# mll-lab-nu/TStar

Measured on AMD Instinct MI355X. Metric: candidate frames scored/sec (whole node) + sec/video to 8 keyframes, 1h@1fps, higher is better.
Workload: dtype f32 held exactly as 3 bf16 terms per operand: every GEMM and vision-attention operand (activations, weights, Q, K, V, softmax probabilities) = three round-to-nearest bf16 terms carrying all 24 significand bits; the 6 partial products with i + j <= 2 (each exact) on v_mfma_f32_32x32x16_bf16, f32 accu

## Files before the change

tstar_amd/csrc/gemm_f32.hip:

```cpp
#include "common.h"
#include "kernels.h"
#include "prof.h"
#include <type_traits>
#include <utility>

namespace tstar {

constexpr int BK = 32, LDS_LD = BK + 4;

__device__ __forceinline__ void tile_mn(int tile, int mt, int nt, int gm, int& mi, int& ni) {
    if (gm <= 1) { mi = tile / nt; ni = tile - mi * nt; return; }
    const int per = gm * nt;
    const int sp = tile / per, r = tile - sp * per;
    const int left = mt - sp * gm;
    const int rows = left < gm ? left : gm;
    ni = r / rows;
    mi = sp * gm + (r - ni * rows);
}

__device__ __forceinline__ float epi_act(float v, int act) {
    if (act == ACT_QGELU) return v * __builtin_amdgcn_rcpf(1.0f + __builtin_amdgcn_exp2f(-1.702f * 1.44269504088896340736f * v));
    if (act == ACT_GELU) return 0.5f * v * (1.0f + erff(v * 0.70710678118654752440f));
    return v;
}

template <int TM_, int TN_, int MINW_>
struct Cfg { static constexpr int TM = TM_, TN = TN_, MINW = MINW_, BM = 2 * TM_ * 32, BN = 2 * TN_ * 32; };
using Cfg128 = Cfg<2, 2, 2>;
using Cfg64N = Cfg<1, 2, 2>;
using Cfg64 = Cfg<1, 1, 4>;
using Cfg128W = Cfg<2, 4, 2>;

template <class CF, int ACT, bool HAS_BIAS, bool HAS_RES, bool PATCH, bool GUARD>
__device__ __forceinline__ void gemm_epilogue_impl(const GemmArgs& g, f32x16 (&acc)[CF::TM][CF::TN], const int m0, const int n0,
                                                   const int wm, const int wn, const int l31, const int h) {
    constexpr int TM = CF::TM, TN = CF::TN;
#pragma unroll
    for (int j = 0; j < TN; ++j) {
        const int col = n0 + wn * TN * 32 + j * 32 + l31;
        const float bv = HAS_BIAS ? g.bias[col] : 0.f;
#pragma unroll
        for (int i = 0; i < TM; ++i) {
            const int rbase = m0 + wm * TM * 32 + i * 32 + 4 * h;
            size_t off[16];
            float extra[16];
#pragma unroll
            for (int r = 0; r < 16; ++r) {
                int row = rbase + (r & 3) + 8 * (r >> 2);
                if (GUARD) row = row < g.M ? row : g.M - 1;
                size_t orow = row;
                float e = 0.f;
                if (PATCH) {
                    const int b = row / g.patch_np, p = row - b * g.patch_np;
                    orow = (size_t)b * (g.patch_np + 1) + 1 + p;
                    e = g.pos[(size_t)(1 + p) * g.N + col];
                }
                off[r] = orow * g.ldc + col;
                if (HAS_RES) e += g.res[off[r]];
                extra[r] = e;
            }
            float v[16];
#pragma unroll
            for (int r = 0; r < 16; ++r) {
                v[r] = epi_act(acc[i][j][r] + bv, ACT);
                if (PATCH || HAS_RES) v[r] += extra[r];
            }
#pragma unroll
            for (int r = 0; r < 16; ++r) {
                if (!GUARD || rbase + (r & 3) + 8 * (r >> 2) < g.M) g.C[off[r]] = v[r];
            }
        }
    }
}

template <class CF, int ACT, bool HAS_BIAS, bool HAS_RES, bool PATCH, bool GUARD>
__device__ __forceinline__ void gemm_epilogue_wide(const GemmArgs& g, f32x16 (&acc)[CF::TM][CF::TN], const int m0, const int n0,
                                                   const int wm, const int wn, const int l31, const int h) {
    constexpr int TM = CF::TM, TN = CF::TN;
#pragma unroll
    for (int i = 0; i < TM; ++i) {
        const int rbase = m0 + wm * TM * 32 + i * 32 + 4 * h;
        unsigned roff[16], poff[PATCH ? 16 : 1];
#pragma unroll
        for (int r = 0; r < 16; ++r) {
            int row = rbase + (r & 3) + 8 * (r >> 2);
            if (GUARD) row = row < g.M ? row : g.M - 1;
            unsigned orow = (unsigned)row;
            if (PATCH) {
                const int b = row / g.patch_np, p = row - b * g.patch_np;
                orow = (unsigned)(b * (g.patch_np + 1) + 1 + p);
                poff[r] = (unsigned)(1 + p) * (unsigned)g.N;
            }
            roff[r] = orow * (unsigned)g.ldc;
        }
#pragma unroll
        for (int j = 0; j < TN; ++j) {
            const int col = n0 + wn * TN * 32 + j * 32 + l31;
            const float bv = HAS_BIAS ? g.bias[col] : 0.f;
            float e[16];
#pragma unroll
            for (int r = 0; r < 16; ++r) {
                float x = 0.f;
                if (PATCH) x = g.pos[(size_t)poff[r] + col];
                if (HAS_RES) x += g.res[(size_t)roff[r] + col];
                e[r] = x;
            }
#pragma unroll
            for (int r = 0; r < 16; ++r) {
                float v = epi_act(acc[i][j][r] + bv, ACT);
                if (PATCH || HAS_RES) v += e[r];
                e[r] = v;
            }
#pragma unroll
            for (int r = 0; r < 16; ++r) {
                if (!GUARD || rbase + (r & 3) + 8 * (r >> 2) < g.M) g.C[(size_t)roff[r] + col] = e[r];
            }
            __builtin_amdgcn_sched_barrier(0);
        }
    }
}

template <class CF, int ACT, bool HAS_BIAS, bool HAS_RES, bool PATCH>
__device__ __forceinline__ void gemm_epilogue(const GemmArgs& g, f32x16 (&acc)[CF::TM][CF::TN], const int m0, const int n0,
                                              const int wm, const int wn, const int l31, const int h) {
    if constexpr (CF::TN >= 4) {
        if (m0 + CF::BM <= g.M) gemm_epilogue_wide<CF, ACT, HAS_BIAS, HAS_RES, PATCH, false>(g, acc, m0, n0, wm, wn, l31, h);
        else gemm_epilogue_wide<CF, ACT, HAS_BIAS, HAS_RES, PATCH, true>(g, acc, m0, n0, wm, wn, l31, h);
        return;
    }
    if (m0 + CF::BM <= g.M) gemm_epilogue_impl<CF, ACT, HAS_BIAS, HAS_RES, PATCH, false>(g, acc, m0, n0, wm, wn, l31, h);
    else gemm_epilogue_impl<CF, ACT, HAS_BIAS, HAS_RES, PATCH, true>(g, acc, m0, n0, wm, wn, l31, h);
}

typedef __bf16 bf16x8 __attribute__((ext_vector_type(8)));
typedef unsigned int u32x4 __attribute__((ext_vector_type(4)));
typedef unsigned int u32x2 __attribute__((ext_vector_type(2)));

__device__ __forceinline__ int bfw_off(int row, int chunk) { return row * 64 + ((chunk ^ ((row >> 2) & 3)) << 4); }

__device__ __forceinline__ void split4_bf16x3(const f32x4 v, u32x2 (&out)[3]) {
    unsigned t[3][4];
#pragma unroll
    for (int e = 0; e < 4; ++e) {
        float r = v[e];
#pragma unroll
        for (int k = 0; k < 3; ++k) {
            const unsigned b = __float_as_uint(r) & 0xFFFF0000u;
            t[k][e] = b;
            r = r - __uint_as_float(b);
        }
    }
#pragma unroll
    for (int k = 0; k < 3; ++k) {
        out[k][0] = (t[k][0] >> 16) | t[k][1];
        out[k][1] = (t[k][2] >> 16) | t[k][3];
    }
}

typedef __bf16 bf16x2 __attribute__((ext_vector_type(2)));
typedef float f32x2 __attribute__((ext_vector_type(2)));
__device__ __forceinline__ void split4_bf16x2(const f32x4 v, u32x2 (&out)[2]) {
#pragma unroll
    for (int p = 0; p < 2; ++p) {
        f32x2 x; x[0] = v[2 * p]; x[1] = v[2 * p + 1];
        const bf16x2 hi = __builtin_convertvector(x, bf16x2);
        const unsigned hb = __builtin_bit_cast(unsigned, hi);
        f32x2 r;
        r[0] = x[0] - __uint_as_float(hb << 16);
        r[1] = x[1] - __uint_as_float(hb & 0xFFFF0000u);
        const bf16x2 lo = __builtin_convertvector(r, bf16x2);
        out[0][p] = hb;
        out[1][p] = __builtin_bit_cast(unsigned, lo);
    }
}

template <class CF, int WMODE, int ACT, bool HAS_BIAS, bool HAS_RES, bool PATCH>
__device__ __forceinline__ void gemm_tile_bf16w(const GemmArgs& g, const int m0, const int n0, float* smem_f) {
    constexpr int TM = CF::TM, TN = CF::TN, BM = CF::BM, BN = CF::BN;
    constexpr int NAT = WMODE == GEMM_W_BF16_EXACT ? 3 : 2, NWT = 1;
    constexpr int NPROD = WMODE == GEMM_W_BF16_2T ? 2 : 3;
    constexpr int DEPTH = TN >= 4 ? 1 : 2;
    constexpr int A_T = BM * 64, W_T = BN * 64, BUF = NAT * A_T + NWT * W_T;
    char* smem = reinterpret_cast<char*>(smem_f);
    const int t = threadIdx.x;
    const int lane = t & 63, wave = t >> 6;
    const int wm = wave >> 1, wn = wave & 1;
    const int l31 = lane & 31, h = lane >> 5;
    constexpr int NA = BM / 32, NB = BN / 64;
    const int c4 = t & 7, r0 = t >> 3;
    const int wc = t & 3, wr = t >> 2;
    const float* ap[NA];
    size_t bo[NB];
#pragma unroll
    for (int i = 0; i < NA; ++i) {
        int ar = m0 + r0 + 32 * i;
        ar = ar < g.M ? ar : g.M - 1;
        ap[i] = g.A + (size_t)ar * g.lda + c4 * 4;
    }
#pragma unroll
    for (int i = 0; i < NB; ++i) bo[i] = (size_t)(n0 + wr + 64 * i) * g.K + wc * 8;

    f32x16 acc[TM][TN];
#pragma unroll
    for (int i = 0; i < TM; ++i)
#pragma unroll
        for (int j = 0; j < TN; ++j)
#pragma unroll
            for (int r = 0; r < 16; ++r) acc[i][j][r] = 0.f;

    f32x4 ra[DEPTH][NA];
    u32x4 rb[DEPTH][NWT][NB];
    auto gload = [&](auto SET, int kt) __attribute__((always_inline)) {
        constexpr int st = decltype(SET)::value;
#pragma unroll
        for (int i = 0; i < NA; ++i) ra[st][i] = *reinterpret_cast<const f32x4*>(ap[i] + kt * BK);
#pragma unroll
        for (int i = 0; i < NB; ++i) {
            rb[st][0][i] = *reinterpret_cast<const u32x4*>(g.Wb + bo[i] + kt * BK);
        }
    };
    auto lstore = [&](auto SET, int buf) __attribute__((always_inline)) {
        constexpr int st = decltype(SET)::value;
        char* base = smem + buf * BUF;
#pragma unroll
        for (int i = 0; i < NA; ++i) {
            u32x2 sp[NAT];
            if constexpr (WMODE == GEMM_W_BF16_EXACT) split4_bf16x3(ra[st][i], sp);
            else split4_bf16x2(ra[st][i], sp);
            const int off = bfw_off(r0 + 32 * i, c4 >> 1) + (c4 & 1) * 8;
#pragma unroll
            for (int k = 0; k < NAT; ++k) *reinterpret_cast<u32x2*>(base + k * A_T + off) = sp[k];
        }
#pragma unroll
        for (int w = 0; w < NWT; ++w)
#pragma unroll
            for (int i = 0; i < NB; ++i)
                *reinterpret_cast<u32x4*>(base + NAT * A_T + w * W_T + bfw_off(wr + 64 * i, wc)) = rb[st][w][i];
    };
    auto compute = [&](int buf) __attribute__((always_inline)) {
        const char* base = smem + buf * BUF;
        __builtin_amdgcn_s_setprio(1);
#pragma unroll
        for (int s = 0; s < 2; ++s) {
            bf16x8 fa[NAT][TM], fw[NWT][TN];
#pragma unroll
            for (int k = 0; k < NAT; ++k)
#pragma unroll
                for (int i = 0; i < TM; ++i)
                    fa[k][i] = *reinterpret_cast<const bf16x8*>(base + k * A_T + bfw_off(wm * TM * 32 + i * 32 + l31, 2 * s + h));
#pragma unroll
            for (int w = 0; w < NWT; ++w)
#pragma unroll
                for (int j = 0; j < TN; ++j)
                    fw[w][j] = *reinterpret_cast<const bf16x8*>(base + NAT * A_T + w * W_T + bfw_off(wn * TN * 32 + j * 32 + l31, 2 * s + h));
#pragma unroll
            for (int p = NPROD - 1; p >= 0; --p) {
                const int ka = p, kw = 0;
#pragma unroll
                for (int i = 0; i < TM; ++i)
#pragma unroll
                    for (int j = 0; j < TN; ++j)
                        acc[i][j] = __builtin_amdgcn_mfma_f32_32x32x16_bf16(fa[ka][i], fw[kw][j], acc[i][j], 0, 0, 0);
            }
        }
        __builtin_amdgcn_s_setprio(0);
    };
    using S0 = std::integral_constant<int, 0>;
    using S1 = std::integral_constant<int, DEPTH - 1>;
    const int nk = g.K / BK;
    if constexpr (DEPTH == 1) {
        gload(S0{}, 0);
        lstore(S0{}, 0);
        __syncthreads();
        for (int kt = 0; kt < nk; ++kt) {
            const bool more = kt + 1 < nk;
            if (more) gload(S0{}, kt + 1);
            compute(kt & 1);
            if (more) lstore(S0{}, (kt + 1) & 1);
            __syncthreads();
        }
        gemm_epilogue<CF, ACT, HAS_BIAS, HAS_RES, PATCH>(g, acc, m0, n0, wm, wn, l31, h);
        return;
    }
    gload(S0{}, 0);
    if (nk > 1) gload(std::integral_constant<int, DEPTH - 1>{}, 1);
    lstore(S0{}, 0);
    __syncthreads();
    for (int kt = 0; kt < nk; kt += 2) {
        if (kt + 2 < nk) gload(S0{}, kt + 2);
        compute(0);
        if (kt + 1 < nk) lstore(S1{}, 1);
        __syncthreads();
        if (kt + 1 >= nk) break;
        if (kt + 3 < nk) gload(S1{}, kt + 3);
        compute(1);
        if (kt + 2 < nk) lstore(S0{}, 0);
        __syncthreads();
    }
    gemm_epilogue<CF, ACT, HAS_BIAS, HAS_RES, PATCH>(g, acc, m0, n0, wm, wn, l31, h);
}

template <int NA>
__device__ __forceinline__ void split4_rn(const f32x4 v, u32x2 (&out)[NA]) {
#pragma unroll
    for (int p = 0; p < 2; ++p) {
        f32x2 x; x[0] = v[2 * p]; x[1] = v[2 * p + 1];
#pragma unroll
        for (int k = 0; k < NA; ++k) {
            const bf16x2 b = __builtin_convertvector(x, bf16x2);
            const unsigned hb = __builtin_bit_cast(unsigned, b);
            out[k][p] = hb;
            if (k + 1 < NA) {
                x[0] = x[0] - __uint_as_float(hb << 16);
                x[1] = x[1] - __uint_as_float(hb & 0xFFFF0000u);
            }
        }
    }
}

__device__ __forceinline__ void split2_rn3(float x0, float x1, unsigned (&o)[3]) {
#pragma unroll
    for (int k = 0; k < 3; ++k) {
        f32x2 x; x[0] = x0; x[1] = x1;
        const unsigned hb = __builtin_bit_cast(unsigned, __builtin_convertvector(x, bf16x2));
        o[k] = hb;
        if (k < 2) {
            x0 = x0 - __uint_as_float(hb << 16);
            x1 = x1 - __uint_as_float(hb & 0xFFFF0000u);
        }
    }
}

template <class CF, int ACT, bool HAS_BIAS, bool HAS_RES, bool PATCH>
__device__ __forceinline__ void gemm_tile_x3(const GemmArgs& g, const int m0, const int n0, float* smem_f) {
    constexpr int TM = CF::TM, TN = CF::TN, BM = CF::BM;
    constexpr int A_T = BM * 64, BUF = 3 * A_T;
    constexpr int NA = BM / 32;
    constexpr int PAIR = TN >= 2 ? 2 : 1, GP = TN / PAIR;
    constexpr int WD = TM * TN == 1 ? 4 : 1;
    static_assert(TN % PAIR == 0, "column tiles go in pairs");
    char* smem = reinterpret_cast<char*>(smem_f);
    const int t = threadIdx.x;
    const int lane = t & 63, wave = __builtin_amdgcn_readfirstlane(t >> 6);
    const int wm = wave >> 1, wn = wave & 1;
    const int l31 = lane & 31, h = lane >> 5;
    const int c4 = t & 7, r0 = t >> 3;
    unsigned aoff[NA];
#pragma unroll
    for (int i = 0; i < NA; ++i) {
        int ar = m0 + r0 + 32 * i;
        ar = ar < g.M ? ar : g.M - 1;
        aoff[i] = (unsigned)(ar - m0) * (unsigned)g.lda * 4u + c4 * 16;
    }
    const int nsteps = g.K / 16, nk = g.K / BK;
    const char* wrow = static_cast<const char*>(g.Wp) + (size_t)((n0 >> 5) + wn * TN) * nsteps * 3072;
    const __amdgpu_buffer_rsrc_t ra_rsrc =
        __builtin_amdgcn_make_buffer_rsrc(const_cast<float*>(g.A + (size_t)m0 * g.lda), 0, 0x7fffffff, 0x00020000);
    const __amdgpu_buffer_rsrc_t rw_rsrc = __builtin_amdgcn_make_buffer_rsrc(const_cast<char*>(wrow), 0, 0x7fffffff, 0x00020000);
    const int voff = lane * 16;
    const int rd0 = (wm * TM * 32 + l31) * 64 + ((h ^ ((l31 >> 2) & 3)) << 4);
    const int rd1 = rd0 ^ 32;
    const int wr0 = r0 * 64 + (((c4 >> 1) ^ ((r0 >> 2) & 3)) << 4) + (c4 & 1) * 8;

    f32x16 acc[TM][TN];
#pragma unroll
    for (int i = 0; i < TM; ++i)
#pragma unroll
        for (int j = 0; j < TN; ++j)
#pragma unroll
            for (int r = 0; r < 16; ++r) acc[i][j][r] = 0.f;

    f32x4 ra[NA];
    u32x4 w[WD][3][TN];
    bf16x8 a0[2][TM], a1[TM], a2[TM];
    unsigned sp[2][3];

    auto gload_a = [&](int kt) __attribute__((always_inline)) {
        kt = kt < nk ? kt : nk - 1;
#pragma unroll
        for (int i = 0; i < NA; ++i)
            ra[i] = __builtin_bit_cast(f32x4, __builtin_amdgcn_raw_buffer_load_b128(ra_rsrc, (int)aoff[i], kt * (BK * 4), 0));
    };
    auto wload = [&](auto SL, auto KW, auto J, int gs) __attribute__((always_inline)) {
        constexpr int sl = decltype(SL)::value, kw = decltype(KW)::value, j = decltype(J)::value;
        gs = gs < nsteps ? gs : nsteps - 1;
        w[sl][kw][j] = __builtin_amdgcn_raw_buffer_load_b128(rw_rsrc, voff + (2 - kw) * 1024, (j * nsteps + gs) * 3072, 0);
    };
    auto rd_a = [&](const char* base, int off, int plane, int i) __attribute__((always_inline)) {
        return *reinterpret_cast<const bf16x8*>(base + off + plane * A_T + i * 2048);
    };
    auto stage_piece = [&](auto P, char* wbase) __attribute__((always_inline)) {
        constexpr int p = decltype(P)::value, i = p >> 1, hf = p & 1;
        split2_rn3(ra[i][2 * hf], ra[i][2 * hf + 1], sp[hf]);
        if constexpr (hf == 1) {
#pragma unroll
            for (int k = 0; k < 3; ++k) {
                u32x2 v; v[0] = sp[0][k]; v[1] = sp[1][k];
                *reinterpret_cast<u32x2*>(wbase + wr0 + k * A_T + i * 2048) = v;
            }
        }
    };
    auto mf = [&](const bf16x8& a, const u32x4& b, f32x16& c) __attribute__((always_inline)) {
        c = __builtin_amdgcn_mfma_f32_32x32x16_bf16(a, __builtin_bit_cast(bf16x8, b), c, 0, 0, 0);
    };
    auto step = [&](auto SS, auto SLOT, const char* rbase, int roff, char* wbase, int gnext, int ktload) __attribute__((always_inline)) {
        constexpr int S = decltype(SS)::value;
        using SL = decltype(SLOT);
        auto& ws = w[SL::value];
        constexpr int NPIECE = NA * 2, NG = 6 * GP, PPG = (NPIECE + 1 + NG - 1) / NG;
        auto after_group = [&](auto G) __attribute__((always_inline)) {
            constexpr int gi = decltype(G)::value;
            if constexpr (S == 0) {
                [&]<int... Q>(std::integer_sequence<int, Q...>) __attribute__((always_inline)) {
                    ([&] {
                        constexpr int p = gi * PPG + Q;
                        if constexpr (p < NPIECE) stage_piece(std::integral_constant<int, p>{}, wbase);
                        if constexpr (p == NPIECE) gload_a(ktload);
                    }(), ...);
                }(std::make_integer_sequence<int, PPG>{});
            }
            if constexpr (gi == 0) {
#pragma unroll
                for (int i = 0; i < TM; ++i) a0[S ^ 1][i] = rd_a(rbase, roff, 0, i);
            }
            __builtin_amdgcn_sched_barrier(0);
        };
        [&]<int... JP>(std::integer_sequence<int, JP...>) __attribute__((always_inline)) {
            ([&] {
                constexpr int j0 = PAIR * JP;
#pragma unroll
                for (int jj = 0; jj < PAIR; ++jj)
#pragma unroll
                    for (int i = 0; i < TM; ++i) mf(a2[i], ws[0][j0 + jj], acc[i][j0 + jj]);
                after_group(std::integral_constant<int, 3 * JP + 0>{});
#pragma unroll
                for (int jj = 0; jj < PAIR; ++jj)
#pragma unroll
                    for (int i = 0; i < TM; ++i) mf(a1[i], ws[0][j0 + jj], acc[i][j0 + jj]);
                after_group(std::integral_constant<int, 3 * JP + 1>{});
#pragma unroll
                for (int jj = 0; jj < PAIR; ++jj)
#pragma unroll
                    for (int i = 0; i < TM; ++i) mf(a0[S][i], ws[0][j0 + jj], acc[i][j0 + jj]);
                [&]<int... JJ>(std::integer_sequence<int, JJ...>) __attribute__((always_inline)) {
                    (wload(SL{}, std::integral_constant<int, 0>{}, std::integral_constant<int, j0 + JJ>{}, gnext), ...);
                }(std::make_integer_sequence<int, PAIR>{});
                after_group(std::integral_constant<int, 3 * JP + 2>{});
            }(), ...);
        }(std::make_integer_sequence<int, GP>{});
#pragma unroll
        for (int i = 0; i < TM; ++i) a2[i] = rd_a(rbase, roff, 2, i);
        __builtin_amdgcn_sched_barrier(0);
        [&]<int... JP>(std::integer_sequence<int, JP...>) __attribute__((always_inline)) {
            ([&] {
                constexpr int j0 = PAIR * JP;
#pragma unroll
                for (int jj = 0; jj < PAIR; ++jj)
#pragma unroll
                    for (int i = 0; i < TM; ++i) mf(a1[i], ws[1][j0 + jj], acc[i][j0 + jj]);
                after_group(std::integral_constant<int, 3 * GP + 2 * JP + 0>{});
#pragma unroll
                for (int jj = 0; jj < PAIR; ++jj)
#pragma unroll
                    for (int i = 0; i < TM; ++i) mf(a0[S][i], ws[1][j0 + jj], acc[i][j0 + jj]);
                [&]<int... JJ>(std::integer_sequence<int, JJ...>) __attribute__((always_inline)) {
                    (wload(SL{}, std::integral_constant<int, 1>{}, std::integral_constant<int, j0 + JJ>{}, gnext), ...);
                }(std::make_integer_sequence<int, PAIR>{});
                after_group(std::integral_constant<int, 3 * GP + 2 * JP + 1>{});
            }(), ...);
        }(std::make_integer_sequence<int, GP>{});
#pragma unroll
        for (int i = 0; i < TM; ++i) a1[i] = rd_a(rbase, roff, 1, i);
        __builtin_amdgcn_sched_barrier(0);
        [&]<int... JP>(std::integer_sequence<int, JP...>) __attribute__((always_inline)) {
            ([&] {
                constexpr int j0 = PAIR * JP;
#pragma unroll
                for (int jj = 0; jj < PAIR; ++jj)
#pragma unroll
                    for (int i = 0; i < TM; ++i) mf(a0[S][i], ws[2][j0 + jj], acc[i][j0 + jj]);
                [&]<int... JJ>(std::integer_sequence<int, JJ...>) __attribute__((always_inline)) {
                    (wload(SL{}, std::integral_constant<int, 2>{}, std::integral_constant<int, j0 + JJ>{}, gnext), ...);
                }(std::make_integer_sequence<int, PAIR>{});
                after_group(std::integral_constant<int, 5 * GP + JP>{});
            }(), ...);
        }(std::make_integer_sequence<int, GP>{});
    };

    gload_a(0);
    [&]<int... Q>(std::integer_sequence<int, Q...>) __attribute__((always_inline)) {
        ((wload(std::integral_constant<int, Q / TN>{}, std::integral_constant<int, 0>{}, std::integral_constant<int, Q % TN>{}, Q / TN),
          wload(std::integral_constant<int, Q / TN>{}, std::integral_constant<int, 1>{}, std::integral_constant<int, Q % TN>{}, Q / TN),
          wload(std::integral_constant<int, Q / TN>{}, std::integral_constant<int, 2>{}, std::integral_constant<int, Q % TN>{}, Q / TN)), ...);
    }(std::make_integer_sequence<int, WD * TN>{});
    [&]<int... P>(std::integer_sequence<int, P...>) __attribute__((always_inline)) {
        (stage_piece(std::integral_constant<int, P>{}, smem), ...);
    }(std::make_integer_sequence<int, NA * 2>{});
    gload_a(1);
    __syncthreads();
#pragma unroll
    for (int i = 0; i < TM; ++i) { a0[0][i] = rd_a(smem, rd0, 0, i); a1[i] = rd_a(smem, rd0, 1, i); a2[i] = rd_a(smem, rd0, 2, i); }
    __builtin_amdgcn_s_setprio(1);
    __builtin_amdgcn_sched_barrier(0);
    auto tile = [&](auto SL0, int kt) __attribute__((always_inline)) {
        constexpr int s0 = decltype(SL0)::value;
        char* cur = smem + (kt & 1) * BUF;
        char* nxt = smem + ((kt + 1) & 1) * BUF;
        step(std::integral_constant<int, 0>{}, std::integral_constant<int, s0>{}, cur, rd1, nxt, 2 * kt + WD, kt + 2);
        asm volatile("s_waitcnt lgkmcnt(0)" ::: "memory");
        __builtin_amdgcn_s_barrier();
        __builtin_amdgcn_sched_barrier(0);
        step(std::integral_constant<int, 1>{}, std::integral_constant<int, (s0 + 1) % WD>{}, nxt, rd0, nxt, 2 * kt + 1 + WD, 0);
    };
    if constexpr (WD <= 2) {
        for (int kt = 0; kt < nk; ++kt) tile(std::integral_constant<int, 0>{}, kt);
    } else {
        static_assert(WD == 4, "the loop below is unrolled by WD / 2 = 2 K tiles");
        int kt = 0;
        for (; kt + 1 < nk; kt += 2) {
            tile(std::integral_constant<int, 0>{}, kt);
            tile(std::integral_constant<int, 2>{}, kt + 1);
        }
        if (kt < nk) tile(std::integral_constant<int, 0>{}, kt);
    }
    __builtin_amdgcn_s_setprio(0);
    gemm_epilogue<CF, ACT, HAS_BIAS, HAS_RES, PATCH>(g, acc, m0, n0, wm, wn, l31, h);
}

__global__ __launch_bounds__(256) void pack_x3_kernel(const float* __restrict__ W, char* __restrict__ Wp, int N, int K) {
    const size_t gid = (size_t)blockIdx.x * 256 + threadIdx.x;
    const int kc = K / 8;
    if (gid >= (size_t)N * kc) return;
    const int n = (int)(gid / kc), c = (int)(gid % kc);
    const f32x4 v0 = *reinterpret_cast<const f32x4*>(W + (size_t)n * K + c * 8);
    const f32x4 v1 = *reinterpret_cast<const f32x4*>(W + (size_t)n * K + c * 8 + 4);
    u32x2 s0[3], s1[3];
    split4_rn<3>(v0, s0);
    split4_rn<3>(v1, s1);
    const int ks = c >> 1, hh = c & 1, nph = (K / 16) * 3;
#pragma unroll
    for (int ph = 0; ph < 3; ++ph) {
        u32x4 o;
        o[0] = s0[2 - ph][0]; o[1] = s0[2 - ph][1]; o[2] = s1[2 - ph][0]; o[3] = s1[2 - ph][1];
        *reinterpret_cast<u32x4*>(Wp + (((size_t)(n >> 5) * nph + ks * 3 + ph) * 64 + hh * 32 + (n & 31)) * 16) = o;
    }
}

int pack_weights_x3(const float* W, void* Wp, int N, int K, hipStream_t s) {
    TSTAR_REQUIRE(N % 32 == 0 && K % 16 == 0, "pack_weights_x3: N must be a multiple of 32, K of 16");
    const size_t n = (size_t)N * (K / 8);
    hipLaunchKernelGGL(pack_x3_kernel, dim3((unsigned)((n + 255) / 256)), dim3(256), 0, s, W, static_cast<char*>(Wp), N, K);
    TSTAR_HIP_CHECK(hipGetLastError());
    return TSTAR_OK;
}

template <class CF, int ACT, bool HAS_BIAS, bool HAS_RES, bool PATCH>
__device__ __forceinline__ void gemm_tile_w2v(const GemmArgs& g, const int m0, const int n0, float* smem_f) {
    constexpr int TM = CF::TM, TN = CF::TN, BM = CF::BM;
    static_assert(TN % 2 == 0, "column tiles go in pairs");
    constexpr int A_T = BM * 64, BUF = 2 * A_T;
    constexpr int NA = BM / 32;
    char* smem = reinterpret_cast<char*>(smem_f);
    const int t = threadIdx.x;
    const int lane = t & 63, wave = __builtin_amdgcn_readfirstlane(t >> 6);
    const int wm = wave >> 1, wn = wave & 1;
    const int l31 = lane & 31, h = lane >> 5;
    const int c4 = t & 7, r0 = t >> 3;
    unsigned aoff[NA];
#pragma unroll
    for (int i = 0; i < NA; ++i) {
        int ar = m0 + r0 + 32 * i;
        ar = ar < g.M ? ar : g.M - 1;
        aoff[i] = (unsigned)(ar - m0) * (unsigned)g.lda * 4u + c4 * 16;
    }
    const int nsteps = g.K / 16, nk = g.K / BK;
    const char* wrow = static_cast<const char*>(g.Wq) + (size_t)((n0 >> 5) + wn * TN) * nsteps * 1024;
    const __amdgpu_buffer_rsrc_t ra_rsrc =
        __builtin_amdgcn_make_buffer_rsrc(const_cast<float*>(g.A + (size_t)m0 * g.lda), 0, 0x7fffffff, 0x00020000);
    const __amdgpu_buffer_rsrc_t rw_rsrc = __builtin_amdgcn_make_buffer_rsrc(const_cast<char*>(wrow), 0, 0x7fffffff, 0x00020000);
    const int voff = lane * 16;
    const int rd0 = (wm * TM * 32 + l31) * 64 + ((h ^ ((l31 >> 2) & 3)) << 4);
    const int rd1 = rd0 ^ 32;
    const int wr0 = r0 * 64 + (((c4 >> 1) ^ ((r0 >> 2) & 3)) << 4) + (c4 & 1) * 8;

    f32x16 acc[TM][TN];
#pragma unroll
    for (int i = 0; i < TM; ++i)
#pragma unroll
        for (int j = 0; j < TN; ++j)
#pragma unroll
            for (int r = 0; r < 16; ++r) acc[i][j][r] = 0.f;
    f32x4 ra[NA];
    u32x4 w[2][TN];
    bf16x8 a0[2][TM], a1[TM];
    unsigned sp[2][2];

    auto gload_a = [&](int kt) __attribute__((always_inline)) {
        kt = kt < nk ? kt : nk - 1;
#pragma unroll
        for (int i = 0; i < NA; ++i)
            ra[i] = __builtin_bit_cast(f32x4, __builtin_amdgcn_raw_buffer_load_b128(ra_rsrc, (int)aoff[i], kt * (BK * 4), 0));
    };
    auto wload = [&](auto SET, auto J, int gs) __attribute__((always_inline)) {
        constexpr int st = decltype(SET)::value, j = decltype(J)::value;
        gs = gs < nsteps ? gs : nsteps - 1;
        w[st][j] = __builtin_amdgcn_raw_buffer_load_b128(rw_rsrc, voff, (j * nsteps + gs) * 1024, 0);
    };
    auto rd_a = [&](const char* base, int off, int plane, int i) __attribute__((always_inline)) {
        return *reinterpret_cast<const bf16x8*>(base + off + plane * A_T + i * 2048);
    };
    auto split_pair = [&](float x0, float x1, unsigned (&o)[2]) __attribute__((always_inline)) {
        f32x2 x; x[0] = x0; x[1] = x1;
        const unsigned hb = __builtin_bit_cast(unsigned, __builtin_convertvector(x, bf16x2));
        o[0] = hb;
        f32x2 r; r[0] = x0 - __uint_as_float(hb << 16); r[1] = x1 - __uint_as_float(hb & 0xFFFF0000u);
        o[1] = __builtin_bit_cast(unsigned, __builtin_convertvector(r, bf16x2));
    };
    auto stage_piece = [&](auto P, char* wbase) __attribute__((always_inline)) {
        constexpr int p = decltype(P)::value, i = p >> 1, hf = p & 1;
        split_pair(ra[i][2 * hf], ra[i][2 * hf + 1], sp[hf]);
        if constexpr (hf == 1) {
#pragma unroll
            for (int k = 0; k < 2; ++k) {
                u32x2 v; v[0] = sp[0][k]; v[1] = sp[1][k];
                *reinterpret_cast<u32x2*>(wbase + wr0 + k * A_T + i * 2048) = v;
            }
        }
    };
    auto mf = [&](const bf16x8& a, const u32x4& b, f32x16& c) __attribute__((always_inline)) {
        c = __builtin_amdgcn_mfma_f32_32x32x16_bf16(a, __builtin_bit_cast(bf16x8, b), c, 0, 0, 0);
    };
    auto step = [&](auto SS, const char* rbase, int roff, char* wbase, int gs, int ktload) __attribute__((always_inline)) {
        constexpr int S = decltype(SS)::value;
        constexpr int NPIECE = NA * 2, GP = TN / 2, NG = 2 * GP, PPG = (NPIECE + 1 + NG - 1) / NG;
        auto after_group = [&](auto G) __attribute__((always_inline)) {
            constexpr int gi = decltype(G)::value;
            if constexpr (S == 0) {
                [&]<int... Q>(std::integer_sequence<int, Q...>) __attribute__((always_inline)) {
                    ([&] {
                        constexpr int p = gi * PPG + Q;
                        if constexpr (p < NPIECE) stage_piece(std::integral_constant<int, p>{}, wbase);
                        if constexpr (p == NPIECE) gload_a(ktload);
                    }(), ...);
                }(std::make_integer_sequence<int, PPG>{});
            }
            if constexpr (gi == 0) {
#pragma unroll
                for (int i = 0; i < TM; ++i) a0[S ^ 1][i] = rd_a(rbase, roff, 0, i);
            }
            __builtin_amdgcn_sched_barrier(0);
        };
        [&]<int... JP>(std::integer_sequence<int, JP...>) __attribute__((always_inline)) {
            ([&] {
                constexpr int j0 = 2 * JP;
#pragma unroll
                for (int jj = 0; jj < 2; ++jj)
#pragma unroll
                    for (int i = 0; i < TM; ++i) mf(a1[i], w[S][j0 + jj], acc[i][j0 + jj]);
                after_group(std::integral_constant<int, 2 * JP + 0>{});
#pragma unroll
                for (int jj = 0; jj < 2; ++jj)
#pragma unroll
                    for (int i = 0; i < TM; ++i) mf(a0[S][i], w[S][j0 + jj], acc[i][j0 + jj]);
                wload(std::integral_constant<int, S>{}, std::integral_constant<int, j0>{}, gs + 2);
                wload(std::integral_constant<int, S>{}, std::integral_constant<int, j0 + 1>{}, gs + 2);
                if constexpr (JP == GP - 1) {
#pragma unroll
                    for (int i = 0; i < TM; ++i) a1[i] = rd_a(rbase, roff, 1, i);
                }
                after_group(std::integral_constant<int, 2 * JP + 1>{});
            }(), ...);
        }(std::make_integer_sequence<int, GP>{});
    };

    gload_a(0);
    [&]<int... J>(std::integer_sequence<int, J...>) __attribute__((always_inline)) {
        ((wload(std::integral_constant<int, 0>{}, std::integral_constant<int, J>{}, 0),
          wload(std::integral_constant<int, 1>{}, std::integral_constant<int, J>{}, 1)), ...);
    }(std::make_integer_sequence<int, TN>{});
    [&]<int... P>(std::integer_sequence<int, P...>) __attribute__((always_inline)) {
        (stage_piece(std::integral_constant<int, P>{}, smem), ...);
    }(std::make_integer_sequence<int, NA * 2>{});
    gload_a(1);
    __syncthreads();
#pragma unroll
    for (int i = 0; i < TM; ++i) { a0[0][i] = rd_a(smem, rd0, 0, i); a1[i] = rd_a(smem, rd0, 1, i); }
    __builtin_amdgcn_s_setprio(1);
    __builtin_amdgcn_sched_barrier(0);
    for (int kt = 0; kt < nk; ++kt) {
        char* cur = smem + (kt & 1) * BUF;
        char* nxt = smem + ((kt + 1) & 1) * BUF;
        step(std::integral_constant<int, 0>{}, cur, rd1, nxt, 2 * kt, kt + 2);
        asm volatile("s_waitcnt lgkmcnt(0)" ::: "memory");
        __builtin_amdgcn_s_barrier();
        __builtin_amdgcn_sched_barrier(0);
        step(std::integral_constant<int, 1>{}, nxt, rd0, nxt, 2 * kt + 1, 0);
    }
    __builtin_amdgcn_s_setprio(0);
    gemm_epilogue<CF, ACT, HAS_BIAS, HAS_RES, PATCH>(g, acc, m0, n0, wm, wn, l31, h);
}

__global__ __launch_bounds__(256) void pack_w2_kernel(const __bf16* __restrict__ Wb, char* __restrict__ Wq, int N, int K) {
    const size_t gid = (size_t)blockIdx.x * 256 + threadIdx.x;
    const int kc = K / 8;
    if (gid >= (size_t)N * kc) return;
    const int n = (int)(gid / kc), c = (int)(gid % kc);
    const u32x4 v = *reinterpret_cast<const u32x4*>(Wb + (size_t)n * K + c * 8);
    const int ks = c >> 1, hh = c & 1;
    *reinterpret_cast<u32x4*>(Wq + (((size_t)(n >> 5) * (K / 16) + ks) * 64 + hh * 32 + (n & 31)) * 16) = v;
}

int pack_weights_w2(const __bf16* Wb, void* Wq, int N, int K, hipStream_t s) {
    TSTAR_REQUIRE(N % 32 == 0 && K % 16 == 0, "pack_weights_w2: N must be a multiple of 32, K of 16");
    const size_t n = (size_t)N * (K / 8);
    hipLaunchKernelGGL(pack_w2_kernel, dim3((unsigned)((n + 255) / 256)), dim3(256), 0, s, Wb, static_cast<char*>(Wq), N, K);
    TSTAR_HIP_CHECK(hipGetLastError());
    return TSTAR_OK;
}

int build_weight_planes(const float* d_W, int N, int K, int wmode, bool want_w2_packed, hipStream_t s, WeightPlanes* out) {
    *out = WeightPlanes();
    TSTAR_REQUIRE(wmode == GEMM_W_F32 || wmode == GEMM_W_BF16_EXACT || wmode == GEMM_W_BF16_2T || wmode == GEMM_W_F32X3, "build_weight_planes: unknown weight mode");
    WeightPlanes p;
    p.wmode = wmode; p.N = N; p.K = K;
    const size_t n = (size_t)N * K;
    if (wmode == GEMM_W_F32X3) {
        TSTAR_HIP_CHECK(hipMalloc(&p.Wp, n * 6));
        RC(pack_weights_x3(d_W, p.Wp, N, K, s));
    } else if (wmode != GEMM_W_F32) {
        TSTAR_HIP_CHECK(hipMalloc(&p.Wb, n * sizeof(__bf16)));
        RC(convert_f32_to_bf16(d_W, p.Wb, nullptr, n, s));
        if (wmode == GEMM_W_BF16_2T && want_w2_packed && w2_plane_shape_ok(N, K)) {
            TSTAR_HIP_CHECK(hipMalloc(&p.Wq, n * sizeof(__bf16)));
            RC(pack_weights_w2(p.Wb, p.Wq, N, K, s));
        }
    }
    *out = std::move(p);
    return TSTAR_OK;
}

template <class CF, int ACT, bool HAS_BIAS, bool HAS_RES, bool PATCH>
__device__ __forceinline__ void gemm_tile(const GemmArgs& g, const int m0, const int n0, float* smem) {
    constexpr int TM = CF::TM, TN = CF::TN, BM = CF::BM, BN = CF::BN;
    float* As = smem;
    float* Bs = smem + 2 * BM * LDS_LD;

    const int t = threadIdx.x;
    const int lane = t & 63, wave = t >> 6;
    const int wm = wave >> 1, wn = wave & 1;
    const int l31 = lane & 31, h = lane >> 5;

    constexpr int NA = BM / 32, NB = BN / 32;
    const int c4 = t & 7, r0 = t >> 3;
    const float* ap[NA];
    const float* bp[NB];
#pragma unroll
    for (int i = 0; i < NA; ++i) {
        int ar = m0 + r0 + 32 * i;
        ar = ar < g.M ? ar : g.M - 1;
        ap[i] = g.A + (size_t)ar * g.lda + c4 * 4;
    }
#pragma unroll
    for (int i = 0; i < NB; ++i) bp[i] = g.W + (size_t)(n0 + r0 + 32 * i) * g.K + c4 * 4;

    f32x16 acc[TM][TN];
#pragma unroll
    for (int i = 0; i < TM; ++i)
#pragma unroll
        for (int j = 0; j < TN; ++j)
#pragma unroll
            for (int r = 0; r < 16; ++r) acc[i][j][r] = 0.f;

    f32x4 ra[NA], rb[NB];
#pragma unroll
    for (int i = 0; i < NA; ++i) ra[i] = *reinterpret_cast<const f32x4*>(ap[i]);
#pragma unroll
    for (int i = 0; i < NB; ++i) rb[i] = *reinterpret_cast<const f32x4*>(bp[i]);
#pragma unroll
    for (int i = 0; i < NA; ++i) *reinterpret_cast<f32x4*>(&As[(r0 + 32 * i) * LDS_LD + c4 * 4]) = ra[i];
#pragma unroll
    for (int i = 0; i < NB; ++i) *reinterpret_cast<f32x4*>(&Bs[(r0 + 32 * i) * LDS_LD + c4 * 4]) = rb[i];
    __syncthreads();

    const int nk = g.K / BK;
    int cur = 0;
    for (int kt = 0; kt < nk; ++kt) {
        const bool more = kt + 1 < nk;
        if (more) {
#pragma unroll
            for (int i = 0; i < NA; ++i) ra[i] = *reinterpret_cast<const f32x4*>(ap[i] + (kt + 1) * BK);
#pragma unroll
            for (int i = 0; i < NB; ++i) rb[i] = *reinterpret_cast<const f32x4*>(bp[i] + (kt + 1) * BK);
        }
        const float* Ac = As + cur * BM * LDS_LD + (wm * TM * 32 + l31) * LDS_LD + h * 4;
        const float* Bc = Bs + cur * BN * LDS_LD + (wn * TN * 32 + l31) * LDS_LD + h * 4;
        __builtin_amdgcn_s_setprio(1);
#pragma unroll
        for (int kk = 0; kk < BK / 8; ++kk) {
            f32x4 fa[TM], fb[TN];
#pragma unroll
            for (int i = 0; i < TM; ++i) fa[i] = *reinterpret_cast<const f32x4*>(Ac + i * 32 * LDS_LD + kk * 8);
#pragma unroll
            for (int j = 0; j < TN; ++j) fb[j] = *reinterpret_cast<const f32x4*>(Bc + j * 32 * LDS_LD + kk * 8);
#pragma unroll
            for (int s = 0; s < 4; ++s)
#pragma unroll
                for (int i = 0; i < TM; ++i)
#pragma unroll
                    for (int j = 0; j < TN; ++j)
                        acc[i][j] = __builtin_amdgcn_mfma_f32_32x32x2f32(fa[i][s], fb[j][s], acc[i][j], 0, 0, 0);
        }
        __builtin_amdgcn_s_setprio(0);
        if (more) {
            float* Aw = As + (cur ^ 1) * BM * LDS_LD;
            float* Bw = Bs + (cur ^ 1) * BN * LDS_LD;
#pragma unroll
            for (int i = 0; i < NA; ++i) *reinterpret_cast<f32x4*>(&Aw[(r0 + 32 * i) * LDS_LD + c4 * 4]) = ra[i];
#pragma unroll
            for (int i = 0; i < NB; ++i) *reinterpret_cast<f32x4*>(&Bw[(r0 + 32 * i) * LDS_LD + c4 * 4]) = rb[i];
        }
        __syncthreads();
        cur ^= 1;
    }

    gemm_epilogue<CF, ACT, HAS_BIAS, HAS_RES, PATCH>(g, acc, m0, n0, wm, wn, l31, h);
}
// ... 216 lines not shown
```

Measured before the change: 12290.

## Peel last K tile and prefetch residual/pos epilogue loads under final MFMAs

For GEMMs with a residual or position-embedding epilogue, the last K tile is peeled. It skips useless next-tile loads and barriers, and issues the first sub-tile's residual/pos loads during the final MFMA groups. The epilogue becomes software-pipelined, loading the next sub-tile's extra operands before storing the current one. The patch row mapping is also simplified to row + row/np + 1. This is meant to hide epilogue global-load latency behind compute, at the cost of more live registers and code complexity.

```diff
diff --git a/tstar_amd/csrc/gemm_f32.hip b/tstar_amd/csrc/gemm_f32.hip
--- a/tstar_amd/csrc/gemm_f32.hip
+++ b/tstar_amd/csrc/gemm_f32.hip
@@ -31,91 +31,154 @@
 using Cfg64 = Cfg<1, 1, 4>;
 using Cfg128W = Cfg<2, 4, 2>;
 
-template <class CF, int ACT, bool HAS_BIAS, bool HAS_RES, bool PATCH, bool GUARD>
-__device__ __forceinline__ void gemm_epilogue_impl(const GemmArgs& g, f32x16 (&acc)[CF::TM][CF::TN], const int m0, const int n0,
-                                                   const int wm, const int wn, const int l31, const int h) {
+template <class CF> using epi_off_t = std::conditional_t<(CF::TN >= 4), unsigned, size_t>;
+
+template <class OFF> struct EpiBand { OFF roff[16]; };
+struct EpiSub { float e[16]; float bv; };
+template <class CF> struct EpiFirst { EpiBand<epi_off_t<CF>> band; EpiSub sub; };
+
+__device__ __forceinline__ size_t epi_idx(unsigned off, int col) { return (size_t)(off + (unsigned)col); }
+__device__ __forceinline__ size_t epi_idx(size_t off, int col) { return off + col; }
+
+template <bool CLAMP>
+__device__ __forceinline__ int epi_row(const GemmArgs& g, const int rbase, const int r) {
+    const int row = rbase + (r & 3) + 8 * (r >> 2);
+    return CLAMP ? (row < g.M ? row : g.M - 1) : row;
+}
+
+template <class OFF, bool PATCH, bool CLAMP>
+__device__ __forceinline__ void epi_band(const GemmArgs& g, const int rbase, EpiBand<OFF>& bd) {
+#pragma unroll
+    for (int r = 0; r < 16; ++r) {
+        const int row = epi_row<CLAMP>(g, rbase, r);
+        if (PATCH) bd.roff[r] = (OFF)(row + row / g.patch_np + 1);
+        else bd.roff[r] = (OFF)row * (OFF)g.ldc;
+    }
+}
+
+template <class OFF, bool HAS_BIAS, bool HAS_RES, bool PATCH, bool CLAMP>
+__device__ __forceinline__ void epi_load(const GemmArgs& g, EpiBand<OFF>& bd, const int rbase, const int col, EpiSub& sb) {
+    static_assert(!(HAS_RES && PATCH), "one extra term per element: the residual or the position row");
+    sb.bv = HAS_BIAS ? g.bias[col] : 0.f;
+#pragma unroll
+    for (int r = 0; r < 16; ++r) {
+        if (PATCH) {
+            const int row = epi_row<CLAMP>(g, rbase, r);
+            const int b = (int)bd.roff[r] - row - 1, p1 = row + 1 - b * g.patch_np;
+            sb.e[r] = g.pos[epi_idx((OFF)p1 * (OFF)g.N, col)];
+        }
+        if (HAS_RES) sb.e[r] = g.res[epi_idx(bd.roff[r], col)];
+    }
+#pragma unroll
+    for (int r = 0; r < 16; ++r) asm volatile("" : "+v"(bd.roff[r]));
+}
+
+template <class OFF, int ACT, bool HAS_RES, bool PATCH, bool GUARD>
+__device__ __forceinline__ void epi_store(const GemmArgs& g, const EpiBand<OFF>& bd, const int rbase, const int col,
+                                          const f32x16& acc, const EpiSub& sb) {
+    float v[16];
+#pragma unroll
+    for (int r = 0; r < 16; ++r) {
+        v[r] = epi_act(acc[r] + sb.bv, ACT);
+        if (PATCH) v[r] += sb.e[r];
+        if (HAS_RES) v[r] += 0.f + sb.e[r];
+    }
+#pragma unroll
+    for (int r = 0; r < 16; ++r) {
+        if (!GUARD || rbase + (r & 3) + 8 * (r >> 2) < g.M) g.C[epi_idx(PATCH ? bd.roff[r] * (OFF)g.ldc : bd.roff[r], col)] = v[r];
+    }
+}
+
+template <class CF, bool HAS_BIAS, bool HAS_RES, bool PATCH>
+__device__ __forceinline__ void gemm_epilogue_first(const GemmArgs& g, const int m0, const int n0, const int wm, const int wn,
+                                                    const int l31, const int h, EpiFirst<CF>& f) {
+    const int rb0 = m0 + wm * CF::TM * 32 + 4 * h;
+    epi_band<epi_off_t<CF>, PATCH, true>(g, rb0, f.band);
+    epi_load<epi_off_t<CF>, HAS_BIAS, HAS_RES, PATCH, true>(g, f.band, rb0, n0 + wn * CF::TN * 32 + l31, f.sub);
+}
+
+template <class CF, int ACT, bool HAS_BIAS, bool HAS_RES, bool PATCH, bool GUARD, bool PRE>
+__device__ __forceinline__ void gemm_epilogue_pipe(const GemmArgs& g, f32x16 (&acc)[CF::TM][CF::TN], const int m0, const int n0,
+                                                   const int wm, const int wn, const int l31, const int h, EpiFirst<CF>& f) {
+    constexpr int TM = CF::TM, TN = CF::TN, NS = TM * TN;
+    static_assert(TM <= 2, "two bands: the first sub-tile's and one more");
+    using OFF = epi_off_t<CF>;
+    EpiBand<OFF> band1;
+    EpiSub sub1;
+    auto band = [&](int i) __attribute__((always_inline)) -> EpiBand<OFF>& { return i == 0 ? f.band : band1; };
+    auto sub = [&](int s) __attribute__((always_inline)) -> EpiSub& { return (s & 1) == 0 ? f.sub : sub1; };
+    int rb0 = m0 + wm * TM * 32 + 4 * h, c0 = n0 + wn * TN * 32 + l31;
+    if constexpr (GUARD) asm volatile("; guarded epilogue" : "+v"(c0), "+v"(rb0));
+    else asm volatile("; unguarded epilogue" : "+v"(c0), "+v"(rb0));
+    if constexpr (!PRE) {
+        epi_band<OFF, PATCH, GUARD>(g, rb0, f.band);
+        epi_load<OFF, HAS_BIAS, HAS_RES, PATCH, GUARD>(g, f.band, rb0, c0, f.sub);
+    }
+    __builtin_amdgcn_sched_barrier(0);
+#pragma unroll
+    for (int s = 0; s < NS; ++s) {
+        if (s + 1 < NS) {
+            const int i1 = (s + 1) / TN, j1 = (s + 1) % TN;
+            if (j1 == 0) epi_band<OFF, PATCH, GUARD>(g, rb0 + i1 * 32, band(i1));
+            epi_load<OFF, HAS_BIAS, HAS_RES, PATCH, GUARD>(g, band(i1), rb0 + i1 * 32, c0 + j1 * 32, sub(s + 1));
+            __builtin_amdgcn_sched_barrier(0);
+        }
+        epi_store<OFF, ACT, HAS_RES, PATCH, GUARD>(g, band(s / TN), rb0 + (s / TN) * 32, c0 + (s % TN) * 32, acc[s / TN][s % TN], sub(s));
+        __builtin_amdgcn_sched_barrier(0);
+    }
+}
+
+template <class CF, int ACT, bool HAS_BIAS, bool HAS_RES, bool PATCH, bool PRE>
+__device__ __forceinline__ void gemm_epilogue_from(const GemmArgs& g, f32x16 (&acc)[CF::TM][CF::TN], const int m0, const int n0,
+                                                   const int wm, const int wn, const int l31, const int h, EpiFirst<CF>& f) {
+    if (m0 + CF::BM <= g.M) gemm_epilogue_pipe<CF, ACT, HAS_BIAS, HAS_RES, PATCH, false, PRE>(g, acc, m0, n0, wm, wn, l31, h, f);
+    else gemm_epilogue_pipe<CF, ACT, HAS_BIAS, HAS_RES, PATCH, true, PRE>(g, acc, m0, n0, wm, wn, l31, h, f);
+}
+
+template <class CF, int ACT, bool HAS_BIAS, bool GUARD>
+__device__ __forceinline__ void gemm_epilogue_plain(const GemmArgs& g, f32x16 (&acc)[CF::TM][CF::TN], const int m0, const int n0,
+                                                    const int wm, const int wn, const int l31, const int h) {
     constexpr int TM = CF::TM, TN = CF::TN;
-#pragma unroll
-    for (int j = 0; j < TN; ++j) {
-        const int col = n0 + wn * TN * 32 + j * 32 + l31;
-        const float bv = HAS_BIAS ? g.bias[col] : 0.f;
+    if constexpr (TN >= 4) {
 #pragma unroll
         for (int i = 0; i < TM; ++i) {
             const int rbase = m0 + wm * TM * 32 + i * 32 + 4 * h;
-            size_t off[16];
-            float extra[16];
-#pragma unroll
-            for (int r = 0; r < 16; ++r) {
-                int row = rbase + (r & 3) + 8 * (r >> 2);
-                if (GUARD) row = row < g.M ? row : g.M - 1;
-                size_t orow = row;
-                float e = 0.f;
-                if (PATCH) {
-                    const int b = row / g.patch_np, p = row - b * g.patch_np;
-                    orow = (size_t)b * (g.patch_np + 1) + 1 + p;
-                    e = g.pos[(size_t)(1 + p) * g.N + col];
+            unsigned roff[16];
+#pragma unroll
+            for (int r = 0; r < 16; ++r) roff[r] = (unsigned)epi_row<GUARD>(g, rbase, r) * (unsigned)g.ldc;
+#pragma unroll
+            for (int j = 0; j < TN; ++j) {
+                const int col = n0 + wn * TN * 32 + j * 32 + l31;
+                const float bv = HAS_BIAS ? g.bias[col] : 0.f;
+                float e[16];
+#pragma unroll
+                for (int r = 0; r < 16; ++r) e[r] = epi_act(acc[i][j][r] + bv, ACT);
+#pragma unroll
+                for (int r = 0; r < 16; ++r) {
+                    if (!GUARD || rbase + (r & 3) + 8 * (r >> 2) < g.M) g.C[(size_t)roff[r] + col] = e[r];
                 }
-                off[r] = orow * g.ldc + col;
-                if (HAS_RES) e += g.res[off[r]];
-                extra[r] = e;
+                __builtin_amdgcn_sched_barrier(0);
             }
-            float v[16];
-#pragma unroll
-            for (int r = 0; r < 16; ++r) {
-                v[r] = epi_act(acc[i][j][r] + bv, ACT);
-                if (PATCH || HAS_RES) v[r] += extra[r];
-            }
-#pragma unroll
-            for (int r = 0; r < 16; ++r) {
-                if (!GUARD || rbase + (r & 3) + 8 * (r >> 2) < g.M) g.C[off[r]] = v[r];
-            }
-        }
-    }
-}
-
-template <class CF, int ACT, bool HAS_BIAS, bool HAS_RES, bool PATCH, bool GUARD>
-__device__ __forceinline__ void gemm_epilogue_wide(const GemmArgs& g, f32x16 (&acc)[CF::TM][CF::TN], const int m0, const int n0,
-                                                   const int wm, const int wn, const int l31, const int h) {
-    constexpr int TM = CF::TM, TN = CF::TN;
-#pragma unroll
-    for (int i = 0; i < TM; ++i) {
-        const int rbase = m0 + wm * TM * 32 + i * 32 + 4 * h;
-        unsigned roff[16], poff[PATCH ? 16 : 1];
-#pragma unroll
-        for (int r = 0; r < 16; ++r) {
-            int row = rbase + (r & 3) + 8 * (r >> 2);
-            if (GUARD) row = row < g.M ? row : g.M - 1;
-            unsigned orow = (unsigned)row;
-            if (PATCH) {
-                const int b = row / g.patch_np, p = row - b * g.patch_np;
-                orow = (unsigned)(b * (g.patch_np + 1) + 1 + p);
-                poff[r] = (unsigned)(1 + p) * (unsigned)g.N;
-            }
-            roff[r] = orow * (unsigned)g.ldc;
-        }
+        }
+    } else {
 #pragma unroll
         for (int j = 0; j < TN; ++j) {
             const int col = n0 + wn * TN * 32 + j * 32 + l31;
             const float bv = HAS_BIAS ? g.bias[col] : 0.f;
-            float e[16];
-#pragma unroll
-            for (int r = 0; r < 16; ++r) {
-                float x = 0.f;
-                if (PATCH) x = g.pos[(size_t)poff[r] + col];
-                if (HAS_RES) x += g.res[(size_t)roff[r] + col];
-                e[r] = x;
+#pragma unroll
+            for (int i = 0; i < TM; ++i) {
+                const int rbase = m0 + wm * TM * 32 + i * 32 + 4 * h;
+                size_t off[16];
+#pragma unroll
+                for (int r = 0; r < 16; ++r) off[r] = (size_t)epi_row<GUARD>(g, rbase, r) * g.ldc + col;
+                float v[16];
+#pragma unroll
+                for (int r = 0; r < 16; ++r) v[r] = epi_act(acc[i][j][r] + bv, ACT);
+#pragma unroll
+                for (int r = 0; r < 16; ++r) {
+                    if (!GUARD || rbase + (r & 3) + 8 * (r >> 2) < g.M) g.C[off[r]] = v[r];
+                }
             }
-#pragma unroll
-            for (int r = 0; r < 16; ++r) {
-                float v = epi_act(acc[i][j][r] + bv, ACT);
-                if (PATCH || HAS_RES) v += e[r];
-                e[r] = v;
-            }
-#pragma unroll
-            for (int r = 0; r < 16; ++r) {
-                if (!GUARD || rbase + (r & 3) + 8 * (r >> 2) < g.M) g.C[(size_t)roff[r] + col] = e[r];
-            }
-            __builtin_amdgcn_sched_barrier(0);
         }
     }
 }
@@ -123,13 +186,13 @@
 template <class CF, int ACT, bool HAS_BIAS, bool HAS_RES, bool PATCH>
 __device__ __forceinline__ void gemm_epilogue(const GemmArgs& g, f32x16 (&acc)[CF::TM][CF::TN], const int m0, const int n0,
                                               const int wm, const int wn, const int l31, const int h) {
-    if constexpr (CF::TN >= 4) {
-        if (m0 + CF::BM <= g.M) gemm_epilogue_wide<CF, ACT, HAS_BIAS, HAS_RES, PATCH, false>(g, acc, m0, n0, wm, wn, l31, h);
-        else gemm_epilogue_wide<CF, ACT, HAS_BIAS, HAS_RES, PATCH, true>(g, acc, m0, n0, wm, wn, l31, h);
-        return;
-    }
-    if (m0 + CF::BM <= g.M) gemm_epilogue_impl<CF, ACT, HAS_BIAS, HAS_RES, PATCH, false>(g, acc, m0, n0, wm, wn, l31, h);
-    else gemm_epilogue_impl<CF, ACT, HAS_BIAS, HAS_RES, PATCH, true>(g, acc, m0, n0, wm, wn, l31, h);
+    if constexpr (HAS_RES || PATCH) {
+        EpiFirst<CF> f;
+        gemm_epilogue_from<CF, ACT, HAS_BIAS, HAS_RES, PATCH, false>(g, acc, m0, n0, wm, wn, l31, h, f);
+    } else {
+        if (m0 + CF::BM <= g.M) gemm_epilogue_plain<CF, ACT, HAS_BIAS, false>(g, acc, m0, n0, wm, wn, l31, h);
+        else gemm_epilogue_plain<CF, ACT, HAS_BIAS, true>(g, acc, m0, n0, wm, wn, l31, h);
+    }
 }
 
 typedef __bf16 bf16x8 __attribute__((ext_vector_type(8)));
@@ -374,6 +437,8 @@
     u32x4 w[WD][3][TN];
     bf16x8 a0[2][TM], a1[TM], a2[TM];
     unsigned sp[2][3];
+    constexpr bool PEEL = (HAS_RES || PATCH) && TM * TN > 1;
+    EpiFirst<CF> first;
 
     auto gload_a = [&](int kt) __attribute__((always_inline)) {
         kt = kt < nk ? kt : nk - 1;
@@ -403,14 +468,17 @@
     auto mf = [&](const bf16x8& a, const u32x4& b, f32x16& c) __attribute__((always_inline)) {
         c = __builtin_amdgcn_mfma_f32_32x32x16_bf16(a, __builtin_bit_cast(bf16x8, b), c, 0, 0, 0);
     };
-    auto step = [&](auto SS, auto SLOT, const char* rbase, int roff, char* wbase, int gnext, int ktload) __attribute__((always_inline)) {
+    auto step = [&](auto SS, auto SLOT, auto LASTF, const char* rbase, int roff, char* wbase, int gnext, int ktload) __attribute__((always_inline)) {
         constexpr int S = decltype(SS)::value;
+        constexpr bool LAST = decltype(LASTF)::value;
+        constexpr bool NEXT = !(LAST && S == 1);
+        constexpr bool WNEXT = !LAST || S + WD < 2;
         using SL = decltype(SLOT);
         auto& ws = w[SL::value];
         constexpr int NPIECE = NA * 2, NG = 6 * GP, PPG = (NPIECE + 1 + NG - 1) / NG;
         auto after_group = [&](auto G) __attribute__((always_inline)) {
             constexpr int gi = decltype(G)::value;
-            if constexpr (S == 0) {
+            if constexpr (S == 0 && !LAST) {
                 [&]<int... Q>(std::integer_sequence<int, Q...>) __attribute__((always_inline)) {
                     ([&] {
                         constexpr int p = gi * PPG + Q;
@@ -419,10 +487,11 @@
                     }(), ...);
                 }(std::make_integer_sequence<int, PPG>{});
             }
-            if constexpr (gi == 0) {
+            if constexpr (gi == 0 && NEXT) {
 #pragma unroll
                 for (int i = 0; i < TM; ++i) a0[S ^ 1][i] = rd_a(rbase, roff, 0, i);
             }
+            if constexpr (gi == 3 * GP - 1 && !NEXT) gemm_epilogue_first<CF, HAS_BIAS, HAS_RES, PATCH>(g, m0, n0, wm, wn, l31, h, first);
             __builtin_amdgcn_sched_barrier(0);
         };
         [&]<int... JP>(std::integer_sequence<int, JP...>) __attribute__((always_inline)) {
@@ -442,14 +511,18 @@
                 for (int jj = 0; jj < PAIR; ++jj)
 #pragma unroll
                     for (int i = 0; i < TM; ++i) mf(a0[S][i], ws[0][j0 + jj], acc[i][j0 + jj]);
-                [&]<int... JJ>(std::integer_sequence<int, JJ...>) __attribute__((always_inline)) {
-                    (wload(SL{}, std::integral_constant<int, 0>{}, std::integral_constant<int, j0 + JJ>{}, gnext), ...);
-                }(std::make_integer_sequence<int, PAIR>{});
+                if constexpr (WNEXT) {
+                    [&]<int... JJ>(std::integer_sequence<int, JJ...>) __attribute__((always_inline)) {
+                        (wload(SL{}, std::integral_constant<int, 0>{}, std::integral_constant<int, j0 + JJ>{}, gnext), ...);
+                    }(std::make_integer_sequence<int, PAIR>{});
+                }
                 after_group(std::integral_constant<int, 3 * JP + 2>{});
             }(), ...);
         }(std::make_integer_sequence<int, GP>{});
-#pragma unroll
-        for (int i = 0; i < TM; ++i) a2[i] = rd_a(rbase, roff, 2, i);
+        if constexpr (NEXT) {
+#pragma unroll
+            for (int i = 0; i < TM; ++i) a2[i] = rd_a(rbase, roff, 2, i);
+        }
         __builtin_amdgcn_sched_barrier(0);
         [&]<int... JP>(std::integer_sequence<int, JP...>) __attribute__((always_inline)) {
             ([&] {
@@ -463,14 +536,18 @@
                 for (int jj = 0; jj < PAIR; ++jj)
 #pragma unroll
                     for (int i = 0; i < TM; ++i) mf(a0[S][i], ws[1][j0 + jj], acc[i][j0 + jj]);
-                [&]<int... JJ>(std::integer_sequence<int, JJ...>) __attribute__((always_inline)) {
-                    (wload(SL{}, std::integral_constant<int, 1>{}, std::integral_constant<int, j0 + JJ>{}, gnext), ...);
-                }(std::make_integer_sequence<int, PAIR>{});
+                if constexpr (WNEXT) {
+                    [&]<int... JJ>(std::integer_sequence<int, JJ...>) __attribute__((always_inline)) {
+                        (wload(SL{}, std::integral_constant<int, 1>{}, std::integral_constant<int, j0 + JJ>{}, gnext), ...);
+                    }(std::make_integer_sequence<int, PAIR>{});
+                }
                 after_group(std::integral_constant<int, 3 * GP + 2 * JP + 1>{});
             }(), ...);
         }(std::make_integer_sequence<int, GP>{});
-#pragma unroll
-        for (int i = 0; i < TM; ++i) a1[i] = rd_a(rbase, roff, 1, i);
+        if constexpr (NEXT) {
+#pragma unroll
+            for (int i = 0; i < TM; ++i) a1[i] = rd_a(rbase, roff, 1, i);
+        }
         __builtin_amdgcn_sched_barrier(0);
         [&]<int... JP>(std::integer_sequence<int, JP...>) __attribute__((always_inline)) {
             ([&] {
@@ -479,9 +556,11 @@
                 for (int jj = 0; jj < PAIR; ++jj)
 #pragma unroll
                     for (int i = 0; i < TM; ++i) mf(a0[S][i], ws[2][j0 + jj], acc[i][j0 + jj]);
-                [&]<int... JJ>(std::integer_sequence<int, JJ...>) __attribute__((always_inline)) {
-                    (wload(SL{}, std::integral_constant<int, 2>{}, std::integral_constant<int, j0 + JJ>{}, gnext), ...);
-                }(std::make_integer_sequence<int, PAIR>{});
+                if constexpr (WNEXT) {
+                    [&]<int... JJ>(std::integer_sequence<int, JJ...>) __attribute__((always_inline)) {
+                        (wload(SL{}, std::integral_constant<int, 2>{}, std::integral_constant<int, j0 + JJ>{}, gnext), ...);
+                    }(std::make_integer_sequence<int, PAIR>{});
+                }
                 after_group(std::integral_constant<int, 5 * GP + JP>{});
             }(), ...);
         }(std::make_integer_sequence<int, GP>{});
@@ -502,26 +581,39 @@
     for (int i = 0; i < TM; ++i) { a0[0][i] = rd_a(smem, rd0, 0, i); a1[i] = rd_a(smem, rd0, 1, i); a2[i] = rd_a(smem, rd0, 2, i); }
     __builtin_amdgcn_s_setprio(1);
     __builtin_amdgcn_sched_barrier(0);
-    auto tile = [&](auto SL0, int kt) __attribute__((always_inline)) {
+    auto tile = [&](auto SL0, auto LASTF, int kt) __attribute__((always_inline)) {
         constexpr int s0 = decltype(SL0)::value;
+        constexpr bool LAST = decltype(LASTF)::value;
         char* cur = smem + (kt & 1) * BUF;
         char* nxt = smem + ((kt + 1) & 1) * BUF;
-        step(std::integral_constant<int, 0>{}, std::integral_constant<int, s0>{}, cur, rd1, nxt, 2 * kt + WD, kt + 2);
-        asm volatile("s_waitcnt lgkmcnt(0)" ::: "memory");
-        __builtin_amdgcn_s_barrier();
+        step(std::integral_constant<int, 0>{}, std::integral_constant<int, s0>{}, LASTF, cur, rd1, nxt, 2 * kt + WD, kt + 2);
+        if constexpr (!LAST) {
+            asm volatile("s_waitcnt lgkmcnt(0)" ::: "memory");
+            __builtin_amdgcn_s_barrier();
+        }
         __builtin_amdgcn_sched_barrier(0);
-        step(std::integral_constant<int, 1>{}, std::integral_constant<int, (s0 + 1) % WD>{}, nxt, rd0, nxt, 2 * kt + 1 + WD, 0);
-    };
+        step(std::integral_constant<int, 1>{}, std::integral_constant<int, (s0 + 1) % WD>{}, LASTF, nxt, rd0, nxt, 2 * kt + 1 + WD, 0);
+    };
+    using STEADY = std::false_type;
+    if constexpr (PEEL) {
+        using PEELED = std::true_type;
+        static_assert(WD <= 2, "a tile's two steps are slots 0 and (WD == 2) 1");
+        for (int kt = 0; kt + 1 < nk; ++kt) tile(std::integral_constant<int, 0>{}, STEADY{}, kt);
+        tile(std::integral_constant<int, 0>{}, PEELED{}, nk - 1);
+        __builtin_amdgcn_s_setprio(0);
+        gemm_epilogue_from<CF, ACT, HAS_BIAS, HAS_RES, PATCH, true>(g, acc, m0, n0, wm, wn, l31, h, first);
+        return;
+    }
     if constexpr (WD <= 2) {
-        for (int kt = 0; kt < nk; ++kt) tile(std::integral_constant<int, 0>{}, kt);
+        for (int kt = 0; kt < nk; ++kt) tile(std::integral_constant<int, 0>{}, STEADY{}, kt);
     } else {
         static_assert(WD == 4, "the loop below is unrolled by WD / 2 = 2 K tiles");
         int kt = 0;
         for (; kt + 1 < nk; kt += 2) {
-            tile(std::integral_constant<int, 0>{}, kt);
-            tile(std::integral_constant<int, 2>{}, kt + 1);
-        }
-        if (kt < nk) tile(std::integral_constant<int, 0>{}, kt);
+            tile(std::integral_constant<int, 0>{}, STEADY{}, kt);
+            tile(std::integral_constant<int, 2>{}, STEADY{}, kt + 1);
+        }
+        if (kt < nk) tile(std::integral_constant<int, 0>{}, STEADY{}, kt);
     }
     __builtin_amdgcn_s_setprio(0);
     gemm_epilogue<CF, ACT, HAS_BIAS, HAS_RES, PATCH>(g, acc, m0, n0, wm, wn, l31, h);
```

Result: no change. 12310 (median of 6 runs) (+0.2%).
